# nicolaivicol/otto-recommender

Measured on AMD Instinct MI355X. Metric: co-visit pairs/sec + candidates/sec at 220M events, 1/2/4/8 MI355X, higher is better.
Workload: dtype int32; 1 GPU; configs[1]: all 5 co-visitation rules, 220M events, 100k-session files; events=220000079, sessions=13435907, parallelism=files dealt over 1 GPU(s)

## Files before the change

otto-recommender_amd/csrc/abi.hip:

```cpp
#include <cstdarg>
#include <cstdlib>
#include <ctime>
#include <algorithm>
#include <mutex>
#include "prims.h"
#include "covis_kernels.h"
#include "table.h"

using namespace ottohip;

namespace ottohip {
static thread_local char g_err[1024] = "";
void set_error(const char* fmt, ...) {
  va_list ap;
  va_start(ap, fmt);
  vsnprintf(g_err, sizeof g_err, fmt, ap);
  va_end(ap);
}
}

namespace ottohip {
Ctx* ctx_base(ottohip_ctx* c) { return c; }

int ensure_part_stats(const ottohip_table* tc) {
// ... 743 lines not shown
    s2 = ctx->aux;
  }
  const char* pipe_env = getenv("OTTOHIP_SPLIT_PIPE");
  const bool pipe_on = pipe_env && atoi(pipe_env) == 1;
  const char* sched_env = getenv("OTTOHIP_REDUCE_SCHED");
  const bool sched = s2 != nullptr && sched_env && atoi(sched_env) == 1 && !pipe_on && !lds_leaf &&
                     getenv("OTTOHIP_HASH_PROF") == nullptr;
  auto level_err = [&](int set) { return sched ? reinterpret_cast<int*>(lcount + set * LC_WORDS + LC_ERR) : err; };
  hipMemsetAsync(lcount, 0, 2 * LC_WORDS * 8, s);
  k_classify_rows<<<grid_for(Rn), 256, 0, s>>>(row_begin, Rn, P, Lt.WB, TL, level_err(0), row_base);
  const char* hgrid_env = getenv("OTTOHIP_HASH_GRID");
  const int hgrid = hgrid_env ? std::max(0, atoi(hgrid_env)) : -1;
  const int fom = FOhist ? 2 : (FOmir ? 3 : (FOon ? 1 : 0));
  unsigned int* hnext = nullptr;
  if (hgrid != 0) OH_TRY(ws.get("hash_next", 2, &hnext));
  if (hgrid < 0 && !ctx->hash_resident[fom]) {
    int nb = 0;
    hipError_t e = fom == 2   ? hipOccupancyMaxActiveBlocksPerMultiprocessor(&nb, k_agg_hash<2>, AGG_T, 0)
                   : fom == 3 ? hipOccupancyMaxActiveBlocksPerMultiprocessor(&nb, k_agg_hash<3>, AGG_T, 0)
                   : fom == 1 ? hipOccupancyMaxActiveBlocksPerMultiprocessor(&nb, k_agg_hash<1>, AGG_T, 0)
                              : hipOccupancyMaxActiveBlocksPerMultiprocessor(&nb, k_agg_hash<0>, AGG_T, 0);
    if (e != hipSuccess || nb < 1) { set_error("k_agg_hash<%d>: occupancy query failed", fom); return OTTOHIP_EHIP; }
    ctx->hash_resident[fom] = nb * ctx->n_cu;
  }
  bool srcA = true;
  bool drained = false;
  const bool dbg = getenv("OTTOHIP_DEBUG") != nullptr;
  if (dbg) fprintf(stderr, "[ottohip] P=%llu rows=%lld\n", (unsigned long long)P, (long long)Rn);
  uint32_t* wcur0 = w0;
  const bool pipe = s2 != nullptr && !lds_leaf && !dbg && getenv("OTTOHIP_HASH_PROF") == nullptr && pipe_on;
  const uint64_t PIPE_MIN_CHUNKS = getenv("OTTOHIP_SPLIT_PIPE_MIN") ? (uint64_t)atoll(getenv("OTTOHIP_SPLIT_PIPE_MIN")) : 2048;
  unsigned long long done[N_LISTS] = {};
  bool hash_early = false;
  auto launch_hash_range = [&](uint64_t lo, uint64_t hi, uint32_t* wb0, hipStream_t st, Task* ov,
                               unsigned long long* n_ov, unsigned long long* ov_work, int slot) {
    if (hi <= lo) return;
    const int64_t nh = (int64_t)(hi - lo);
    const Task* th = TL.hash + lo;
    const int64_t blocks = hgrid == 0 ? (int64_t)agg_grid : (hgrid > 0 ? (int64_t)hgrid : (int64_t)ctx->hash_resident[fom]);
    const unsigned hg = (unsigned)std::min<int64_t>(nh, blocks);
    unsigned int* nt = hgrid == 0 ? nullptr : hnext + slot;
    if (nt) hipMemsetAsync(nt, 0, sizeof(unsigned int), st);
    if (FOhist)
      k_agg_hash<2><<<hg, AGG_T, 0, st>>>(th, nh, wb0, w1, row_key, R, Lt, n_rules, O, ov, n_ov, fo, nt, ov_work);
    else if (FOmir)
      k_agg_hash<3><<<hg, AGG_T, 0, st>>>(th, nh, wb0, w1, row_key, R, Lt, n_rules, O, ov, n_ov, fo, nt, ov_work);
    else if (FOon)
      k_agg_hash<1><<<hg, AGG_T, 0, st>>>(th, nh, wb0, w1, row_key, R, Lt, n_rules, O, ov, n_ov, fo, nt, ov_work);
    else
      k_agg_hash<<<hg, AGG_T, 0, st>>>(th, nh, wb0, w1, row_key, R, Lt, n_rules, O, ov, n_ov, fo, nt, ov_work);
  };
  auto launch_sorts = [&](const unsigned long long* lo, const unsigned long long* hi, uint32_t* wb0, hipStream_t st) {
    const unsigned sgrid = (unsigned)ctx->n_cu * 32;
#define OH_SORT(c, M)                                                                                          \
    if (hi[c] > lo[c]) {                                                                                       \
      const int64_t n_ = (int64_t)(hi[c] - lo[c]);                                                             \
      const Task* t_ = TL.sort[c] + lo[c];                                                                     \
      const unsigned g_ = (unsigned)std::min<uint64_t>(ceil_div(n_, 4), sgrid);                                \
      if (FOhist)                                                                                              \
        k_agg_sort<M, 2><<<g_, 256, (size_t)fo.nf * 8, st>>>(t_, n_, wb0, w1, row_key, R, Lt, n_rules, Osort, fo); \
      else if (FOmir)                                                                                          \
        k_agg_sort<M, 3><<<g_, 256, 0, st>>>(t_, n_, wb0, w1, row_key, R, Lt, n_rules, Osort, fo);             \
      else if (FOon)                                                                                           \
        k_agg_sort<M, 1><<<g_, 256, 0, st>>>(t_, n_, wb0, w1, row_key, R, Lt, n_rules, Osort, fo);             \
      else                                                                                                     \
        k_agg_sort<M><<<g_, 256, 0, st>>>(t_, n_, wb0, w1, row_key, R, Lt, n_rules, Osort, fo);                \
    }
    OH_SORT(0, 1) OH_SORT(1, 2) OH_SORT(2, 4) OH_SORT(3, 8) OH_SORT(4, 16)
#undef OH_SORT
  };
  static const int sub = getenv("OTTOHIP_SPLIT_SUB") ? atoi(getenv("OTTOHIP_SPLIT_SUB")) : 4096;
  const char* lds_env = getenv("OTTOHIP_SPLIT_LDS");
  const bool split_lds = lds_env ? atoi(lds_env) != 0 : SPLIT_LDS_DEFAULT;
  const char* ldsmin_env = getenv("OTTOHIP_SPLIT_LDS_MIN");
  const uint32_t lds_min = (uint32_t)std::min(SPLIT_CH + 1, std::max(0, ldsmin_env ? atoi(ldsmin_env) : SPLIT_LDS_MIN));
  const int lds_t = getenv("OTTOHIP_SPLIT_LDS_T") ? atoi(getenv("OTTOHIP_SPLIT_LDS_T")) : SPLIT_LT;
  auto scatter_chunks = [&](const Task* cur_split, int64_t ns, const uint64_t* chb, const uint32_t* ctask, const uint64_t* mtb,
                            const uint64_t* hoff, uint32_t* hmat, uint32_t c0, uint32_t c1) {
    if (c1 <= c0) return;
    uint32_t max_len = SPLIT_CH;
    if (split_lds) {
      if (lds_t == 512)
        k_split_scatter_lds<512><<<c1 - c0, 512, 0, s>>>(cur_split, ns, chb, ctask, mtb, hoff, wcur0, w1, Lt.F, hmat, c0, lds_min);
// ... 12 lines not shown
    hipStream_t s3 = ctx->aux2;
    const unsigned long long* hv = ctx->level_host;
    Task* ovl[2] = {nullptr, nullptr};
    bool hash_pending = false;
    for (int level = 0; level < 40; ++level) {
      const int p = level & 1;
      unsigned long long* C = lcount + p * LC_WORDS;
      unsigned long long* Cn = lcount + (p ^ 1) * LC_WORDS;
      wcur0 = (level == 0 || !w2) ? w0 : w2;
      if (hash_pending) OH_HIP(hipStreamWaitEvent(s, ctx->ev_hash, 0));
      hash_pending = false;
      OH_HIP(hipMemcpyAsync(ctx->level_host, C, LC_WORDS * 8, hipMemcpyDeviceToHost, s));
      OH_HIP(hipMemsetAsync(Cn, 0, LC_WORDS * 8, s));
      OH_HIP(hipEventRecord(ctx->ev_fork, s));
      OH_HIP(hipStreamSynchronize(s));
      if (hv[LC_ERR]) {
        set_error("task list overflow / row too large (err=%d)", (int)hv[LC_ERR]);
        return OTTOHIP_ELIMIT;
      }
      unsigned long long nlist[N_LISTS];
      for (int c = 0; c < N_LISTS; ++c) nlist[c] = hv[c];
      const uint64_t nh = nlist[N_SORT], nov = hv[LC_OVERFLOW];
      const int64_t nsl = (int64_t)nlist[N_SORT + 1], ns = nsl + (int64_t)nov;
      const int64_t nchunks = (int64_t)hv[LC_CHUNKS], ndig = (int64_t)hv[LC_DIGITS], nent = (int64_t)hv[LC_ENTRIES];
      if (dbg)
        fprintf(stderr, "[ottohip] level %d: sort %llu/%llu/%llu/%llu/%llu hash %llu split %llu lds %llu overflow %llu "
                "(chunks %lld digits %lld entries %lld)\n", level, nlist[0], nlist[1], nlist[2], nlist[3], nlist[4],
                (unsigned long long)nh, nlist[N_SORT + 1], nlist[N_SORT + 2], (unsigned long long)nov, (long long)nchunks,
                (long long)ndig, (long long)nent);
      if ((uint64_t)nsl > TL.cap) { set_error("split list overflow"); return OTTOHIP_ELIMIT; }
      if (nh) {
        if ((rc = ws.get(p ? "t_overB" : "t_overA", (size_t)nh, &ovl[p]))) return rc;
        OH_HIP(hipStreamWaitEvent(s3, ctx->ev_fork, 0));
        launch_hash_range(0, nh, wcur0, s3, ovl[p], Cn + LC_OVERFLOW, Cn + LC_CHUNKS, 0);
        OH_HIP(hipEventRecord(ctx->ev_hash, s3));
        hash_pending = true;
      }
      OH_HIP(hipStreamWaitEvent(s2, ctx->ev_fork, 0));
      const unsigned long long zero[N_LISTS] = {};
      launch_sorts(zero, nlist, wcur0, s2);
      OH_HIP(hipEventRecord(ctx->ev_join[p], s2));
      if (ns == 0 && !hash_pending) {
        OH_HIP(hipStreamWaitEvent(s, ctx->ev_join[p], 0));
        drained = true;
        return 0;
      }
      Task* cur_split = TL.split;
      uint32_t *nch, *ndg, *nen, *hmat = nullptr;
      uint64_t *chb, *dgb = nullptr, *mtb = nullptr, *tot2, *hoff = nullptr;
      if (ns) {
        if (nov)
          OH_HIP(hipMemcpyAsync(cur_split + nsl, ovl[p ^ 1], (size_t)nov * sizeof(Task), hipMemcpyDeviceToDevice, s));
        uint32_t* ctask;
        if ((rc = ws.get("sp_nch", (size_t)ns, &nch)) || (rc = ws.get("sp_ndg", (size_t)ns, &ndg)) ||
            (rc = ws.get("sp_nen", (size_t)ns, &nen)) || (rc = ws.get("sp_chb", (size_t)ns + 1, &chb)) ||
            (rc = ws.get("sp_dgb", (size_t)ns + 1, &dgb)) || (rc = ws.get("sp_mtb", (size_t)ns + 1, &mtb)) ||
            (rc = ws.get("sp_tot", 6, &tot2)) || (rc = ws.get("sp_hmat", (size_t)nent, &hmat)) ||
            (rc = ws.get("sp_hoff", (size_t)nent + 1, &hoff)) || (rc = ws.get("sp_ctask", (size_t)nchunks, &ctask)))
          return rc;
        k_split_prepare<<<grid_for(ns), 256, 0, s>>>(cur_split, ns, nch, ndg, nen);
        if ((rc = exclusive_scan_u32(ctx, nch, chb, ns, tot2, s)) || (rc = exclusive_scan_u32(ctx, ndg, dgb, ns, tot2 + 1, s)) ||
            (rc = exclusive_scan_u32(ctx, nen, mtb, ns, tot2 + 2, s)))
          return rc;
        k_split_chunk_task<<<grid_for(ns), 256, 0, s>>>(chb, nch, ns, ctask);
        k_split_hist<<<(unsigned)nchunks, SPLIT_T, 0, s>>>(cur_split, ns, chb, ctask, mtb, wcur0, w1, Lt.F, hmat);
        if ((rc = exclusive_scan_u32(ctx, hmat, hoff, nent, hoff + nent, s))) return rc;
        scatter_chunks(cur_split, ns, chb, ctask, mtb, hoff, hmat, 0, (uint32_t)nchunks);
      }
      if (level >= 1) OH_HIP(hipStreamWaitEvent(s, ctx->ev_join[p ^ 1], 0));
      if ((rc = get_lists(std::max(cap0, (uint64_t)ndig), p ? "t_splitA" : "t_splitB", p ^ 1, nh))) return rc;
      TL.n = Cn;
      if (ns) k_split_classify<<<grid_for(ndig), 256, 0, s>>>(cur_split, ns, dgb, mtb, hoff, ndig, TL, level_err(p ^ 1), hmat, 0);
      if (hipGetLastError() != hipSuccess) { set_error("split launch failed"); return OTTOHIP_EHIP; }
    }
    return 0;
  };
  if (sched) OH_TRY(sched_levels());
  for (int level = 0; !sched && level < 40; ++level) {
    wcur0 = (level == 0 || !w2) ? w0 : w2;
    unsigned long long nlist[N_LISTS];
    if ((rc = d2h(nlist, lcount, N_LISTS, s))) return rc;
    if ((rc = d2h(&herr, err, 1, s))) return rc;
    if (herr) { set_error("task list overflow / row too large (err=%d)", herr); return OTTOHIP_ELIMIT; }
    if (dbg) {
      fprintf(stderr, "[ottohip] level %d: sort %llu/%llu/%llu/%llu/%llu hash %llu split %llu lds %llu\n", level, nlist[0],
              nlist[1], nlist[2], nlist[3], nlist[4], nlist[N_SORT], nlist[N_SORT + 1], nlist[N_SORT + 2]);
      Task* lists[N_LISTS] = {TL.sort[0], TL.sort[1], TL.sort[2], TL.sort[3], TL.sort[4], TL.hash, TL.split, TL.lds};
      fprintf(stderr, "[ottohip] level %d words:", level);
      for (int c = 0; c < N_LISTS; ++c) {
        std::vector<Task> tv(nlist[c]);
        if (nlist[c]) (void)d2h(tv.data(), lists[c], nlist[c], s);
        unsigned long long sw = 0, mx = 0;
        for (auto& t : tv) { sw += t.len; mx = std::max<unsigned long long>(mx, t.len); }
        fprintf(stderr, " %llu(max %llu)", sw, mx);
        if (c == N_SORT + 1 && !tv.empty()) {
          unsigned long long hw[40] = {}, hn[40] = {};
          for (auto& t : tv) { const int b = 63 - __builtin_clzll((unsigned long long)t.len | 1ull); hw[b] += t.len; ++hn[b]; }
          fprintf(stderr, " [split by log2 len:");
          for (int b = 0; b < 40; ++b)
            if (hn[b]) fprintf(stderr, " 2^%d:%llu tasks/%llu words", b, hn[b], hw[b]);
          fprintf(stderr, "]");
        }
      }
      fprintf(stderr, "\n");
    }
    hipStream_t ss = s2 ? s2 : s;
    if (s2) { OH_HIP(hipEventRecord(ctx->ev_fork, s)); OH_HIP(hipStreamWaitEvent(s2, ctx->ev_fork, 0)); }
    static const bool hash_first = !(getenv("OTTOHIP_HASH_FIRST") && !strcmp(getenv("OTTOHIP_HASH_FIRST"), "0"));
    const bool hf = hash_first && nlist[N_SORT] > done[N_SORT];
    auto launch_hash = [&]() {
      launch_hash_range(done[N_SORT], nlist[N_SORT], wcur0, s, TL.split, lcount + N_SORT + 1, nullptr, 0);
    };
    if (hf) launch_hash();
    launch_sorts(done, nlist, wcur0, ss);
    if (s2) OH_HIP(hipEventRecord(ctx->ev_join[level & 1], s2));
    if (nlist[N_SORT + 2]) {
      const unsigned lg = (unsigned)std::min<uint64_t>(nlist[N_SORT + 2], (uint64_t)ctx->n_cu * 4);
      if (FOon)
        k_agg_lds<true><<<lg, LDS_T, 0, s>>>(TL.lds, (int64_t)nlist[N_SORT + 2], wcur0, w1, row_key, R, Lt, O, TL.split,
                                             lcount + N_SORT + 1, TL.cap + split_extra, err, fo);
      else
        k_agg_lds<<<lg, LDS_T, 0, s>>>(TL.lds, (int64_t)nlist[N_SORT + 2], wcur0, w1, row_key, R, Lt, O, TL.split,
                                       lcount + N_SORT + 1, TL.cap + split_extra, err, fo);
    }
    if (nlist[N_SORT] > done[N_SORT]) {
      static const bool hprof = getenv("OTTOHIP_HASH_PROF") != nullptr && !hash_first;
      if (hprof) {
        if ((rc = ws.get("hash_prof", (size_t)(2 * nlist[N_SORT]), &fo.prof))) return rc;
        OH_HIP(hipMemsetAsync(fo.prof, 0, 16 * nlist[N_SORT], s));
      }
      if (!hf) launch_hash();
      if (hprof) {
        std::vector<unsigned long long> pv(2 * nlist[N_SORT]);
        if ((rc = d2h(pv.data(), fo.prof, pv.size(), s))) return rc;
        std::vector<size_t> ord(nlist[N_SORT]);
        for (size_t i = 0; i < ord.size(); ++i) ord[i] = i;
        auto tk = [&](size_t i) { return pv[2 * i + 1] & ~(1ull << 63); };
        std::sort(ord.begin(), ord.end(), [&](size_t a, size_t b) { return tk(a) > tk(b); });
        unsigned long long tsum = 0, wsum = 0;
        for (size_t i = 0; i < ord.size(); ++i) { tsum += tk(i); wsum += (uint32_t)pv[2 * i]; }
        fprintf(stderr, "[ottohip] hash level %d: %zu tasks, %llu words, %.3f ms summed task time; slowest:", level,
                ord.size(), wsum, tsum / 1e5);
        for (size_t i = 0; i < ord.size() && i < 10; ++i)
          fprintf(stderr, " [len %u rows %u %.3f ms%s]", (uint32_t)pv[2 * ord[i]], (uint32_t)(pv[2 * ord[i]] >> 32),
                  tk(ord[i]) / 1e5, (pv[2 * ord[i] + 1] >> 63) ? " full" : "");
        fprintf(stderr, "\n");
        fo.prof = nullptr;
      }
    }
    if (hash_early) OH_HIP(hipStreamWaitEvent(s, ctx->ev_hash, 0));
    if (nlist[N_SORT] || nlist[N_SORT + 2])
      if ((rc = d2h(nlist, lcount, N_LISTS, s))) return rc;
    hash_early = false;
    for (int c = 0; c < N_LISTS; ++c) done[c] = 0;
    const int64_t ns = (int64_t)nlist[N_SORT + 1];
    if (dbg) fprintf(stderr, "[ottohip] level %d: split after hash overflow %lld\n", level, (long long)ns);
    if (ns == 0) {
      if (s2) OH_HIP(hipStreamWaitEvent(s, ctx->ev_join[level & 1], 0));
      drained = true;
      break;
    }
    if ((uint64_t)ns > TL.cap) { set_error("split list overflow"); return OTTOHIP_ELIMIT; }
    Task* cur_split = TL.split;
    uint32_t *nch, *ndg, *nen;
    uint64_t *chb, *dgb, *mtb, *tot2;
    if ((rc = ws.get("sp_nch", (size_t)ns, &nch)) || (rc = ws.get("sp_ndg", (size_t)ns, &ndg)) ||
        (rc = ws.get("sp_nen", (size_t)ns, &nen)) || (rc = ws.get("sp_chb", (size_t)ns + 1, &chb)) ||
        (rc = ws.get("sp_dgb", (size_t)ns + 1, &dgb)) || (rc = ws.get("sp_mtb", (size_t)ns + 1, &mtb)) ||
        (rc = ws.get("sp_tot", 6, &tot2)))
      return rc;
    k_split_prepare<<<grid_for(ns), 256, 0, s>>>(cur_split, ns, nch, ndg, nen);
    if ((rc = exclusive_scan_u32(ctx, nch, chb, ns, tot2, s)) || (rc = exclusive_scan_u32(ctx, ndg, dgb, ns, tot2 + 1, s)) ||
        (rc = exclusive_scan_u32(ctx, nen, mtb, ns, tot2 + 2, s)))
      return rc;
    if (pipe) k_split_half<<<1, 64, 0, s>>>(chb, dgb, ns, tot2, tot2 + 3);
    uint64_t tt[6] = {0, 0, 0, 0, 0, 0};
    if ((rc = d2h(tt, tot2, pipe ? 6 : 3, s))) return rc;
    const int64_t nchunks = (int64_t)tt[0], ndig = (int64_t)tt[1], nent = (int64_t)tt[2];
    const bool piped = pipe && (uint64_t)nchunks >= PIPE_MIN_CHUNKS && tt[3] > 0 && (int64_t)tt[3] < ns &&
                       tt[4] > 0 && (int64_t)tt[4] < nchunks && tt[5] > 0 && (int64_t)tt[5] < ndig;
    const uint32_t cA = piped ? (uint32_t)tt[4] : (uint32_t)nchunks;
    const int64_t dA = piped ? (int64_t)tt[5] : ndig;
    uint32_t *hmat, *ctask;
    uint64_t* hoff;
    if ((rc = ws.get("sp_hmat", (size_t)nent, &hmat)) || (rc = ws.get("sp_hoff", (size_t)nent + 1, &hoff)) ||
        (rc = ws.get("sp_ctask", (size_t)nchunks, &ctask)))
      return rc;
    k_split_chunk_task<<<grid_for(ns), 256, 0, s>>>(chb, nch, ns, ctask);
    k_split_hist<<<(unsigned)nchunks, SPLIT_T, 0, s>>>(cur_split, ns, chb, ctask, mtb, wcur0, w1, Lt.F, hmat);
    if ((rc = exclusive_scan_u32(ctx, hmat, hoff, nent, hoff + nent, s))) return rc;
    auto scatter = [&](uint32_t c0, uint32_t c1) { scatter_chunks(cur_split, ns, chb, ctask, mtb, hoff, hmat, c0, c1); };
    scatter(0, cA);
    if (s2 && level >= 1) OH_HIP(hipStreamWaitEvent(s, ctx->ev_join[(level + 1) & 1], 0));
    const uint64_t capn = (uint64_t)ndig;
    if ((rc = get_lists(std::max(cap0, capn), srcA ? "t_splitB" : "t_splitA", (level + 1) & 1))) return rc;
    hipMemsetAsync(lcount, 0, LC_WORDS * 8, s);
    k_split_classify<<<grid_for(dA), 256, 0, s>>>(cur_split, ns, dgb, mtb, hoff, dA, TL, err, hmat, 0);
    if (piped) {
      if (getenv("OTTOHIP_SPLIT_PIPE_LOG")) fprintf(stderr, "[ottohip] level %d split pipelined at chunk %u of %lld\n", level, cA, (long long)nchunks);
      OH_HIP(hipEventRecord(ctx->ev_half, s));
      scatter(cA, (uint32_t)nchunks);
      if (ndig > dA)
        k_split_classify<<<grid_for(ndig - dA), 256, 0, s>>>(cur_split, ns, dgb, mtb, hoff, ndig, TL, err, hmat, dA);
      OH_HIP(hipStreamWaitEvent(ctx->aux2, ctx->ev_half, 0));
      unsigned long long nA[N_LISTS];
      if ((rc = d2h(nA, lcount, N_LISTS, ctx->aux2))) return rc;
      OH_HIP(hipStreamWaitEvent(s2, ctx->ev_half, 0));
      uint32_t* wb0 = w2 ? w2 : w0;
      if (nA[N_SORT]) {
        launch_hash_range(0, nA[N_SORT], wb0, s2, TL.split, lcount + N_SORT + 1, nullptr, 1);
        OH_HIP(hipEventRecord(ctx->ev_hash, s2));
        hash_early = true;
      }
      const unsigned long long zero[N_LISTS] = {};
      launch_sorts(zero, nA, wb0, s2);
      for (int c = 0; c <= N_SORT; ++c) done[c] = nA[c];
    }
    srcA = !srcA;
    if (hipGetLastError() != hipSuccess) { set_error("split launch failed"); return OTTOHIP_EHIP; }
  }
  ctx->end(ph, s);
  if (!drained) { set_error("reduce: split levels did not converge"); return OTTOHIP_ELIMIT; }
  std::vector<unsigned long long> stv((size_t)STAT_STRIPES * STAT_STRIDE);
  if ((rc = d2h(stv.data(), stats, stv.size(), s))) return rc;
  unsigned long long st[STAT_STRIDE] = {};
  for (int k = 0; k < STAT_STRIPES; ++k)
    for (int j = 0; j < STAT_STRIDE; ++j) st[j] += stv[(size_t)k * STAT_STRIDE + j];
  if (hipGetLastError() != hipSuccess) { set_error("reduce failed"); return OTTOHIP_EHIP; }
  unsigned long long U = 0, dropped = 0;
  for (int r = 0; r < n_rules; ++r) U += st[r * 4 + 0];
  const unsigned long long sum_pairs = st[STAT_RAW + 1], raw_rows = st[STAT_RAW];
  if (FOon) {
    if ((rc = d2h(&dropped, fo.dropped, 1, s))) return rc;
    if (fo.dbg) {
      unsigned long long dv[8];
      if ((rc = d2h(dv, fo.dbg, 8, s))) return rc;
      fprintf(stderr, "[ottohip] file opts: hash dropped %llu kept %llu (loaded %llu inserted %llu), sort dropped %llu kept %llu\n",
              dv[0], dv[1], dv[4], dv[5], dv[2], dv[3]);
    }
    if ((rc = file_opts_finish(fopts, fo, s))) return rc;
  }
  T->n_rows = (int64_t)U;
  T->n_slots = (int64_t)n_slots;
// ... 1096 lines not shown
```

otto-recommender_amd/csrc/covis_kernels.h:

```cpp
#pragma once
#include "prims.h"

namespace ottohip {

constexpr int EV_BLOCK = 256;
constexpr int LCAP = 512;
constexpr int SPLIT_MEAN = 420;
constexpr int LDS_SPLIT_MEAN = 2560;
__constant__ uint32_t c_split_mean = SPLIT_MEAN;
__constant__ uint32_t c_split_runs = 0;
__constant__ uint32_t c_split_fuse = 1;
__constant__ uint32_t c_hash_prio = 0;
__constant__ uint32_t c_lds_leaf = 0;
constexpr uint32_t W_EMPTY = 0xFFFFFFFFu;
constexpr int STAT_STRIPES = 256;
constexpr int STAT_RAW = MAX_RULES * 4;
constexpr int STAT_STRIDE = STAT_RAW + 8;

struct RulesDev {
  int32_t lo[MAX_RULES], hi[MAX_RULES];
  uint32_t mask[MAX_RULES];
  int32_t n_of_type[4];
  int32_t rule_of_type[4][MAX_RULES];
  uint32_t sym_mask;
// ... 2196 lines not shown
    }
  }
  return created;
}

constexpr int N_SORT = 5;
constexpr int SORT_MAX = 64 << (N_SORT - 1);
constexpr int LDS_CAP = 4096;
struct TaskLists {
  Task* sort[N_SORT];
  Task* hash;
  Task* split;
  Task* lds;
  unsigned long long* n;
  uint64_t cap;
};
constexpr int N_LISTS = N_SORT + 3;
constexpr int LC_CHUNKS = N_LISTS, LC_DIGITS = N_LISTS + 1, LC_ENTRIES = N_LISTS + 2, LC_OVERFLOW = N_LISTS + 3,
              LC_ERR = N_LISTS + 4, LC_WORDS = 16;
static_assert(LC_ERR < LC_WORDS, "counter set");
__device__ __forceinline__ uint32_t split_ndig_len(uint64_t len);
__device__ __forceinline__ void split_work(uint64_t len, uint32_t& nch, uint32_t& nd) {
  nch = (uint32_t)((len + 16383ull) / 16384ull);
  nd = split_ndig_len(len);
}

template <int FOM = 0>
__global__ __launch_bounds__(AGG_T, 2) void k_agg_hash(const Task* __restrict__ tasks, int64_t n_tasks,
                                                    const uint32_t* __restrict__ w0, const uint32_t* __restrict__ w1,
                                                    const uint32_t* __restrict__ row_key, RulesDev R, Layout L,
                                                    int n_rules, OutRows O, Task* __restrict__ overflow,
                                                    unsigned long long* __restrict__ n_overflow, FileOpts fo,
                                                    unsigned int* __restrict__ next_task = nullptr,
                                                    unsigned long long* __restrict__ ov_work = nullptr) {
  __shared__ unsigned long long lds[2 * HCAP];
  __shared__ unsigned int s_next;
  __shared__ uint32_t wtot[AGG_T / 64];
  __shared__ uint32_t nocc;
  constexpr bool FO = FOM != 0, PM = FOM == 1 || FOM == 3;
  __shared__ unsigned long long fh[FO ? FO_MAXF : 1];
  __shared__ std::conditional_t<PM, PartLds, char> sP[1];
  const int tid = threadIdx.x;
  if (c_hash_prio == 1) __builtin_amdgcn_s_setprio(1);
  else if (c_hash_prio >= 2) __builtin_amdgcn_s_setprio(3);
  RuleAcc acc;
  acc.zero();
  if constexpr (FO) {
    for (uint32_t i = tid; i < fo.nf; i += AGG_T) fh[i] = 0;
    if constexpr (PM) part_lds_load(fo, sP[0]);
    __syncthreads();
  }
  const bool pmode = PM && fo.parts;
  auto take_task = [&](int64_t prev) -> int64_t {
    if (!next_task) return prev < 0 ? (int64_t)blockIdx.x : prev + (int64_t)gridDim.x;
    __syncthreads();
    if (tid == 0) s_next = atomicAdd(next_task, 1u);
    __syncthreads();
    return (int64_t)s_next;
  };
  for (int64_t ti = take_task(-1); ti < n_tasks; ti = take_task(ti)) {
    const Task T = tasks[ti];
    const uint64_t t_start = fo.prof ? wall_clock64() : 0;
    const uint32_t* W = (T.buf ? w1 : w0) + T.begin;
    const RowInfo ri = row_info(row_key, T.row, L.A);
    const bool fo_row = FO && ri.type == fo.type;
    const bool fo_cut = fo_row && (fo.cuts || fo.qonly);
    uint32_t ndrop = 0, dbg_loaded = 0, dbg_ins = 0;
    const uint32_t dbound = T.len;
    const bool optimistic = 2 * dbound > (uint32_t)HCAP;
    uint32_t cap = 64;
    while (cap < 2 * dbound && cap < (uint32_t)HCAP) cap <<= 1;
    const uint32_t cm = cap - 1, limit = (uint32_t)HCAP / 4;
    unsigned long long* A = lds;
    for (uint32_t i = tid; i < cap; i += AGG_T) A[i] = SLOT_EMPTY;
    if (tid == 0) nocc = 0;
    __syncthreads();
    bool full = false;
    constexpr int PF = 8;
    uint32_t wbuf[PF], nbuf[PF];
    const uint32_t l64 = (uint32_t)tid & 63u;
#pragma unroll
    for (int j = 0; j < PF; ++j) {
      const uint32_t i = j * AGG_T + tid;
      nbuf[j] = i < T.len ? W[i] : W_EMPTY;
    }
    for (uint32_t i0 = 0; i0 < T.len && !full; i0 += AGG_T * PF) {
#pragma unroll
      for (int j = 0; j < PF; ++j) {
        wbuf[j] = nbuf[j];
        const uint32_t i = i0 + (uint32_t)(AGG_T * PF) + j * AGG_T + tid;
        nbuf[j] = i < T.len ? W[i] : W_EMPTY;
      }
#pragma unroll
      for (int j = 0; j < PF; ++j) {
        if (FO && fo.dbg && wbuf[j] != W_EMPTY) ++dbg_loaded;
        if constexpr (PM) {
          const bool dr = fo_cut && fo_drop(fo, wbuf[j], ri.aid, L);
          ndrop += dr ? 1u : 0u;
          wbuf[j] = dr ? W_EMPTY : wbuf[j];
        }
      }
      if (optimistic && __hip_atomic_load(&nocc, __ATOMIC_RELAXED, __HIP_MEMORY_SCOPE_WORKGROUP) > limit) {
        full = true;
        break;
      }
      uint32_t inc[PF], slot[PF];
#pragma unroll
      for (int j = 0; j < PF; ++j) {
        const uint32_t w = wbuf[j];
        const bool head = l64 == 0u || lane_prev(w) != w;
        const uint64_t hm = __ballot(head);
        const uint64_t after = l64 == 63u ? 0ull : hm & (~0ull << (l64 + 1u));
        const uint32_t end = after ? (uint32_t)__builtin_ctzll(after) : 64u;
        inc[j] = end - l64;
        wbuf[j] = head ? w : W_EMPTY;
      }
      const uint32_t created = hash_insert_batch<PF>(A, wbuf, inc, cm, slot);
      if (FO && fo.dbg) {
#pragma unroll
        for (int j = 0; j < PF; ++j) dbg_ins += (wbuf[j] != W_EMPTY && slot[j] != HASH_FULL) ? inc[j] : 0u;
      }
#pragma unroll
      for (int j = 0; j < PF; ++j) full |= wbuf[j] != W_EMPTY && slot[j] == HASH_FULL;
      if (optimistic) {
        const uint32_t nc = wave_sum(created);
        if (nc && (tid & 63) == 0) atomicAdd(&nocc, nc);
      }
    }
    full = __syncthreads_or(full);
    if (full) {
      if (tid == 0) {
        const unsigned long long k = atomicAdd(n_overflow, 1ull);
        overflow[k] = T;
        if (ov_work) {
          uint32_t nch, nd;
          split_work(T.len, nch, nd);
          atomicAdd(ov_work + 0, (unsigned long long)nch);
          atomicAdd(ov_work + 1, (unsigned long long)nd);
          atomicAdd(ov_work + 2, (unsigned long long)nch * nd);
        }
        if (fo.prof) {
          fo.prof[2 * ti] = T.len;
          fo.prof[2 * ti + 1] = (wall_clock64() - t_start) | (1ull << 63);
        }
      }
      __syncthreads();
      continue;
    }
    constexpr int SL = HCAP / AGG_T;
    uint32_t kw[SL], kc[SL];
#pragma unroll
    for (int s = 0; s < SL; ++s) {
      const uint32_t slot = tid + s * AGG_T;
      const unsigned long long v = slot < cap ? A[slot] : SLOT_EMPTY;
      kw[s] = (uint32_t)(v >> 32);
      kc[s] = (uint32_t)v;
    }
    if constexpr (FO) {
      const uint32_t nd = wave_sum(ndrop);
      if (nd && (tid & 63) == 0) atomicAdd(fo.dropped, (unsigned long long)nd);
      if (fo.dbg) {
        uint32_t kept = 0;
#pragma unroll
        for (int s = 0; s < SL; ++s) kept += kw[s] != W_EMPTY ? kc[s] : 0u;
        kept = wave_sum(kept);
        const uint32_t ld = wave_sum(dbg_loaded), ins = wave_sum(dbg_ins);
        if ((tid & 63) == 0) {
          atomicAdd(fo.dbg + 0, (unsigned long long)nd); atomicAdd(fo.dbg + 1, (unsigned long long)kept);
          atomicAdd(fo.dbg + 4, (unsigned long long)ld); atomicAdd(fo.dbg + 5, (unsigned long long)ins);
        }
      }
      if (fo.hist && fo_row) {
#pragma unroll
        for (int s = 0; s < SL; ++s)
          if (kw[s] != W_EMPTY && (kw[s] >> (L.A + L.F)) == fo.q) {
            const unsigned long long mult = (fo.sym && ((kw[s] >> L.F) & L.amask) != (uint32_t)ri.aid) ? 2ull : 1ull;
            atomicAdd(&fh[kw[s] & ((1u << L.F) - 1u)], mult * (kc[s] >= 2 ? (1ull | (1ull << 32)) : 1ull));
          }
      }
    }
    __syncthreads();
    const int npass = (FOM == 3 && pmode && fo.mirror_off) ? 2 : 1;
    uint32_t nout = 0;
#pragma unroll 1
    for (int pass = 0; pass < npass; ++pass) {
    unsigned long long* B = lds;
    unsigned long long* B2 = lds + cap;
    for (uint32_t i = tid; i < cap; i += AGG_T) { B[i] = SLOT_EMPTY; B2[i] = 0; }
    __syncthreads();
#pragma unroll
    for (int s0 = 0; s0 < SL; s0 += 8) {
      if ((uint32_t)(s0 * AGG_T) >= cap) break;
      uint32_t k2[8], c8[8], slot[8];
#pragma unroll
      for (int j = 0; j < 8; ++j) {
        k2[j] = kw[s0 + j] == W_EMPTY ? W_EMPTY : kw[s0 + j] >> L.F;
        if constexpr (PM) {
          if (pmode && kw[s0 + j] != W_EMPTY) {
            const uint32_t w = kw[s0 + j], f = w & ((1u << L.F) - 1u), ci = sP[0].cut_of[f];
            const uint64_t ka = (uint64_t)(uint32_t)ri.aid, kb = (uint64_t)((w >> L.F) & L.amask);
            const uint64_t key = pass ? ((kb << 32) | ka) : ((ka << 32) | kb);
            k2[j] |= ((uint32_t)sP[0].part_of[f] +
                      ((ci != FO_NOCUT && key >= sP[0].cut_key[ci & (FO_MAXCUT - 1)]) ? 1u : 0u)) << 24;
          }
        }
        c8[j] = kc[s0 + j];
      }
      hash_insert_batch<8>(B, k2, c8, cm, slot);
#pragma unroll
      for (int j = 0; j < 8; ++j) {
        if (slot[j] == HASH_FULL) continue;
        const uint32_t c = c8[j];
        atomicAdd(&B2[slot[j]], ((unsigned long long)(c >= 2 ? c : 0u) << 32) | 1ull | ((c >= 2 ? 1ull : 0ull) << 16));
      }
    }
    __syncthreads();
    uint32_t mine = 0;
    for (uint32_t i = tid; i < cap; i += AGG_T) {
      const uint32_t k2 = (uint32_t)(B[i] >> 32);
      mine += k2 != W_EMPTY && !(pass && (int32_t)(k2 & L.amask) == ri.aid);
    }
    const uint32_t incl = wave_incl_scan(mine);
    if ((tid & 63) == 63) wtot[tid >> 6] = incl;
    __syncthreads();
    uint32_t pre = 0;
    for (int k = 0; k < (tid >> 6); ++k) pre += wtot[k];
    const uint64_t base = T.begin + (pass ? fo.mirror_off : 0ull);
    uint64_t p = base + pre + incl - mine;
    for (uint32_t i = tid; i < cap; i += AGG_T) {
      const unsigned long long v = B[i];
      const uint32_t k2 = (uint32_t)(v >> 32);
      if (k2 == W_EMPTY) continue;
      const unsigned long long v2 = B2[i];
      const int rule = pmode ? 0 : R.rule_of_type[ri.type][k2 >> L.A];
      const uint32_t c = (uint32_t)v, c2 = (uint32_t)(v2 >> 32), nf = (uint32_t)v2;
      const int32_t next = (int32_t)(k2 & L.amask);
      if (pass) {
        if (next != ri.aid) put_row(O, p++, (int)(k2 >> 24), next, ri.aid, c, c2);
        continue;
      }
      const bool mr = rule_sym(R, rule) && next != ri.aid;
      put_row(O, p++, pmode ? (int)(k2 >> 24) : rule, ri.aid, next, c, c2);
      acc.add(rule, c, nf, mr ? 2u : 1u);
    }
    const uint32_t no = wtot[0] + wtot[1] + wtot[2] + wtot[3];
    for (uint32_t i = no + tid; i < T.len; i += AGG_T) O.rule[base + i] = 0xFF;
    if (pass == 0) nout = no;
    __syncthreads();
    }
    if (fo.prof && tid == 0) {
      fo.prof[2 * ti] = T.len | ((unsigned long long)nout << 32);
      fo.prof[2 * ti + 1] = wall_clock64() - t_start;
    }
  }
  acc.flush(O.stats, n_rules);
  if constexpr (FO) {
    if (fo.hist) {
      __syncthreads();
      for (uint32_t i = tid; i < fo.nf; i += AGG_T)
        if (fh[i]) atomicAdd(&fo.hist[i], fh[i]);
    }
  }
}


constexpr int SPLIT_LEVELS = 4;
__device__ __forceinline__ int task_class(uint64_t len, uint32_t level, bool split) {
  for (int c = 0; c < N_SORT; ++c)
    if (len <= (uint64_t)(64 << c)) return c;
  if (split && c_lds_leaf && len <= (uint64_t)LDS_CAP && level < (uint32_t)SPLIT_LEVELS) return N_SORT + 2;
  return (split && level < (uint32_t)SPLIT_LEVELS) ? N_SORT + 1 : N_SORT;
}
__device__ __forceinline__ void push_task_block(const TaskLists& TL, bool valid, uint64_t begin, uint64_t len,
                                                uint32_t row, uint32_t rem, uint32_t buf, bool split, int* err) {
  __shared__ uint32_t bcnt[N_LISTS];
  __shared__ unsigned long long bbase[N_LISTS];
  __shared__ unsigned long long bwork[3];
  if (valid && len > 0xFFFFFFFFull) { atomicOr(err, 2); valid = false; }
  const int c = valid ? task_class(len, rem, split) : -1;
  if (threadIdx.x < N_LISTS) bcnt[threadIdx.x] = 0;
  if (threadIdx.x < 3) bwork[threadIdx.x] = 0;
  __syncthreads();
  uint32_t my = 0;
#pragma unroll
  for (int q = 0; q < N_LISTS; ++q) {
    const uint64_t m = __ballot(c == q);
    if (!m) continue;
    uint32_t wb = 0;
    if (mbcnt(m) == 0 && c == q) wb = atomicAdd(&bcnt[q], (uint32_t)__popcll(m));
    wb = __shfl(wb, __ffsll((long long)m) - 1);
    if (c == q) my = wb + mbcnt(m);
    if (q == N_SORT + 1) {
      uint32_t nch = 0, nd = 0;
      if (c == q) split_work(len, nch, nd);
// ... 311 lines not shown
    for (uint32_t q = 0; q < (tid >> 6); ++q) pre += wsum[q];
    const uint32_t st = pre + incl - v;
    if (own) g = T.begin + st;
    if (tid < (uint32_t)SPLIT_DMAX) { cur[tid] = st; delta[tid] = g - st; }
  }
  __syncthreads();
  for (uint32_t i0 = 0; i0 < m; i0 += 8 * TB) {
    uint32_t wr[8];
#pragma unroll
    for (int j = 0; j < 8; ++j) {
      const uint32_t i = i0 + tid + j * TB;
      wr[j] = i < m ? Win[i] : 0u;
    }
#pragma unroll
    for (int j = 0; j < 8; ++j) {
      const bool valid = i0 + tid + j * TB < m;
      const uint32_t d = split_digit(wr[j], F, T.rem, nd);
      uint32_t slot;
      if (c_split_runs) slot = lds_add_runs(cur, d, valid);
      else slot = valid ? atomicAdd(&cur[d], 1u) : 0u;
      if (valid && slot < (uint32_t)SPLIT_CH) stage[slot] = wr[j];
    }
  }
  __syncthreads();
  for (uint32_t p = tid; p < m; p += TB) {
    const uint32_t w = stage[p];
    Wout[delta[split_digit(w, F, T.rem, nd)] + p] = w;
  }
}

__global__ void k_split_classify(const Task* __restrict__ tasks, int64_t n, const uint64_t* __restrict__ digit_base,
                                 const uint64_t* __restrict__ mat_base, const uint64_t* __restrict__ hoff,
                                 int64_t n_digits_total, TaskLists TL, int* err, const uint32_t* __restrict__ hmat,
                                 int64_t d0 = 0) {
  const int64_t i = d0 + (int64_t)blockIdx.x * blockDim.x + threadIdx.x;
  Task T;
  T.begin = 0; T.rem = 0; T.row = 0; T.buf = 0; T.len = 0;
  uint64_t b = 0, c = 0;
  if (i < n_digits_total) {
    const int64_t t = find_task(digit_base, n, (uint64_t)i);
    T = tasks[t];
    const uint64_t d = (uint64_t)i - digit_base[t], nch = (uint64_t)ceil_div((int64_t)T.len, SPLIT_CH);
    const uint64_t mb = mat_base[t];
    if (nch == 1 && c_split_fuse) {
      uint64_t lo = 0;
      for (uint64_t e = 0; e < d; ++e) lo += hmat[mb + e];
      c = hmat[mb + d];
      b = T.begin + lo;
    } else {
      const uint64_t lo = hoff[mb + d * nch], hi = hoff[mb + (d + 1) * nch];
      c = hi - lo;
      b = T.begin + (lo - hoff[mb]);
    }
  }
  const bool again = c != 0 && (uint64_t)c <= 4 * ((uint64_t)T.len / split_ndig(T) + 1);
  push_task_block(TL, c != 0, b, c, T.row, T.rem + 1u, T.buf ^ 1u, again, err);
}

constexpr int LDS_T = 256;
constexpr int LDS_WPT = LDS_CAP / LDS_T;
constexpr int LDS_SUBW = 32;
constexpr int LDS_NSUB = LDS_CAP / LDS_SUBW;
constexpr int LDS_SEG = 384;
constexpr int LDS_BIG = 128;
static_assert(LDS_SEG + LDS_BIG <= 512, "a grouped segment fits the 512-word fold");
static_assert(LDS_NSUB <= 128, "sub-bucket scan over waves 0 and 1");
template <bool FO = false>
__global__ __launch_bounds__(LDS_T) void k_agg_lds(const Task* __restrict__ tasks, int64_t n_tasks,
                                                   uint32_t* __restrict__ w0, uint32_t* __restrict__ w1,
                                                   const uint32_t* __restrict__ row_key, RulesDev R, Layout L,
                                                   OutRows O, Task* __restrict__ overflow,
                                                   unsigned long long* __restrict__ n_overflow, uint64_t ov_cap,
                                                   int* __restrict__ err, FileOpts fo) {
  __shared__ uint32_t words[LDS_CAP];
  __shared__ uint32_t sh[LDS_NSUB], ss[LDS_NSUB + 1], seg[LDS_NSUB + 1];
  __shared__ uint32_t wtot[LDS_T / 64], nseg;
  __shared__ unsigned long long sacc[LDS_T / 64][STAT_STRIDE];
  __shared__ RulesDev sR;
  __shared__ uint32_t stg[LDS_T / 64][2][64 * 8 + 64];
  __shared__ unsigned long long fh[FO ? FO_MAXF : 1];
  __shared__ std::conditional_t<FO, PartLds, char> sP[1];
  const int tid = threadIdx.x, wv = tid >> 6;
  const uint32_t l = lane_id();
  if (tid == 0) sR = R;
  for (int i = (int)l; i < STAT_STRIDE; i += 64) sacc[wv][i] = 0;
  if constexpr (FO) {
    for (uint32_t i = tid; i < fo.nf; i += LDS_T) fh[i] = 0;
    part_lds_load(fo, sP[0]);
// ... 803 lines not shown
```

Baseline: 98.09 billion pairs/s.

## Size hash tables to task occupancy, prefetch next hash task, add optional task ordering

```diff
diff --git a/otto-recommender_amd/csrc/abi.hip b/otto-recommender_amd/csrc/abi.hip
--- a/otto-recommender_amd/csrc/abi.hip
+++ b/otto-recommender_amd/csrc/abi.hip
@@ -799,23 +799,40 @@
   const uint64_t PIPE_MIN_CHUNKS = getenv("OTTOHIP_SPLIT_PIPE_MIN") ? (uint64_t)atoll(getenv("OTTOHIP_SPLIT_PIPE_MIN")) : 2048;
   unsigned long long done[N_LISTS] = {};
   bool hash_early = false;
+  const bool hot_hash = getenv("OTTOHIP_HOT_HASH") && !strcmp(getenv("OTTOHIP_HOT_HASH"), "1");
+  const bool hash_order = getenv("OTTOHIP_HASH_ORDER") && !strcmp(getenv("OTTOHIP_HASH_ORDER"), "1");
   auto launch_hash_range = [&](uint64_t lo, uint64_t hi, uint32_t* wb0, hipStream_t st, Task* ov,
-                               unsigned long long* n_ov, unsigned long long* ov_work, int slot) {
-    if (hi <= lo) return;
+                               unsigned long long* n_ov, unsigned long long* ov_work, int slot) -> int {
+    if (hi <= lo) return 0;
     const int64_t nh = (int64_t)(hi - lo);
     const Task* th = TL.hash + lo;
+    const uint32_t* trk = nullptr;
     const int64_t blocks = hgrid == 0 ? (int64_t)agg_grid : (hgrid > 0 ? (int64_t)hgrid : (int64_t)ctx->hash_resident[fom]);
+    if (hash_order && nh > blocks) {
+      Task* sorted;
+      uint32_t* srk;
+      unsigned int* cls;
+      if (int r = ws.get(slot ? "hash_sorted1" : "hash_sorted0", (size_t)nh, &sorted)) return r;
+      if (int r = ws.get(slot ? "hash_rk1" : "hash_rk0", (size_t)nh, &srk)) return r;
+      if (int r = ws.get(slot ? "hash_cls1" : "hash_cls0", 64, &cls)) return r;
+      hipMemsetAsync(cls, 0, 64 * sizeof(unsigned int), st);
+      k_hash_classes<<<grid_for(nh), HORD_T, 0, st>>>(th, nh, cls);
+      k_hash_order<<<grid_for(nh), HORD_T, 0, st>>>(th, nh, row_key, cls, cls + 32, sorted, srk);
+      th = sorted;
+      trk = srk;
+    }
     const unsigned hg = (unsigned)std::min<int64_t>(nh, blocks);
     unsigned int* nt = hgrid == 0 ? nullptr : hnext + slot;
     if (nt) hipMemsetAsync(nt, 0, sizeof(unsigned int), st);
     if (FOhist)
-      k_agg_hash<2><<<hg, AGG_T, 0, st>>>(th, nh, wb0, w1, row_key, R, Lt, n_rules, O, ov, n_ov, fo, nt, ov_work);
+      k_agg_hash<2><<<hg, AGG_T, 0, st>>>(th, nh, wb0, w1, row_key, R, Lt, n_rules, O, ov, n_ov, fo, nt, ov_work, trk);
     else if (FOmir)
-      k_agg_hash<3><<<hg, AGG_T, 0, st>>>(th, nh, wb0, w1, row_key, R, Lt, n_rules, O, ov, n_ov, fo, nt, ov_work);
+      k_agg_hash<3><<<hg, AGG_T, 0, st>>>(th, nh, wb0, w1, row_key, R, Lt, n_rules, O, ov, n_ov, fo, nt, ov_work, trk);
     else if (FOon)
-      k_agg_hash<1><<<hg, AGG_T, 0, st>>>(th, nh, wb0, w1, row_key, R, Lt, n_rules, O, ov, n_ov, fo, nt, ov_work);
+      k_agg_hash<1><<<hg, AGG_T, 0, st>>>(th, nh, wb0, w1, row_key, R, Lt, n_rules, O, ov, n_ov, fo, nt, ov_work, trk);
     else
-      k_agg_hash<<<hg, AGG_T, 0, st>>>(th, nh, wb0, w1, row_key, R, Lt, n_rules, O, ov, n_ov, fo, nt, ov_work);
+      k_agg_hash<<<hg, AGG_T, 0, st>>>(th, nh, wb0, w1, row_key, R, Lt, n_rules, O, ov, n_ov, fo, nt, ov_work, trk);
+    return 0;
   };
   auto launch_sorts = [&](const unsigned long long* lo, const unsigned long long* hi, uint32_t* wb0, hipStream_t st) {
     const unsigned sgrid = (unsigned)ctx->n_cu * 32;
@@ -894,7 +911,7 @@
       if (nh) {
         if ((rc = ws.get(p ? "t_overB" : "t_overA", (size_t)nh, &ovl[p]))) return rc;
         OH_HIP(hipStreamWaitEvent(s3, ctx->ev_fork, 0));
-        launch_hash_range(0, nh, wcur0, s3, ovl[p], Cn + LC_OVERFLOW, Cn + LC_CHUNKS, 0);
+        if ((rc = launch_hash_range(0, nh, wcur0, s3, ovl[p], Cn + LC_OVERFLOW, Cn + LC_CHUNKS, 0))) return rc;
         OH_HIP(hipEventRecord(ctx->ev_hash, s3));
         hash_pending = true;
       }
@@ -932,7 +949,7 @@
       if (level >= 1) OH_HIP(hipStreamWaitEvent(s, ctx->ev_join[p ^ 1], 0));
       if ((rc = get_lists(std::max(cap0, (uint64_t)ndig), p ? "t_splitA" : "t_splitB", p ^ 1, nh))) return rc;
       TL.n = Cn;
-      if (ns) k_split_classify<<<grid_for(ndig), 256, 0, s>>>(cur_split, ns, dgb, mtb, hoff, ndig, TL, level_err(p ^ 1), hmat, 0);
+      if (ns) k_split_classify<<<grid_for(ndig), 256, 0, s>>>(cur_split, ns, dgb, mtb, hoff, ndig, TL, level_err(p ^ 1), hmat, 0, hot_hash);
       if (hipGetLastError() != hipSuccess) { set_error("split launch failed"); return OTTOHIP_EHIP; }
     }
     return 0;
@@ -970,10 +987,10 @@
     if (s2) { OH_HIP(hipEventRecord(ctx->ev_fork, s)); OH_HIP(hipStreamWaitEvent(s2, ctx->ev_fork, 0)); }
     static const bool hash_first = !(getenv("OTTOHIP_HASH_FIRST") && !strcmp(getenv("OTTOHIP_HASH_FIRST"), "0"));
     const bool hf = hash_first && nlist[N_SORT] > done[N_SORT];
-    auto launch_hash = [&]() {
-      launch_hash_range(done[N_SORT], nlist[N_SORT], wcur0, s, TL.split, lcount + N_SORT + 1, nullptr, 0);
+    auto launch_hash = [&]() -> int {
+      return launch_hash_range(done[N_SORT], nlist[N_SORT], wcur0, s, TL.split, lcount + N_SORT + 1, nullptr, 0);
     };
-    if (hf) launch_hash();
+    if (hf && (rc = launch_hash())) return rc;
     launch_sorts(done, nlist, wcur0, ss);
     if (s2) OH_HIP(hipEventRecord(ctx->ev_join[level & 1], s2));
     if (nlist[N_SORT + 2]) {
@@ -991,7 +1008,7 @@
         if ((rc = ws.get("hash_prof", (size_t)(2 * nlist[N_SORT]), &fo.prof))) return rc;
         OH_HIP(hipMemsetAsync(fo.prof, 0, 16 * nlist[N_SORT], s));
       }
-      if (!hf) launch_hash();
+      if (!hf && (rc = launch_hash())) return rc;
       if (hprof) {
         std::vector<unsigned long long> pv(2 * nlist[N_SORT]);
         if ((rc = d2h(pv.data(), fo.prof, pv.size(), s))) return rc;
@@ -1007,6 +1024,12 @@
           fprintf(stderr, " [len %u rows %u %.3f ms%s]", (uint32_t)pv[2 * ord[i]], (uint32_t)(pv[2 * ord[i]] >> 32),
                   tk(ord[i]) / 1e5, (pv[2 * ord[i] + 1] >> 63) ? " full" : "");
         fprintf(stderr, "\n");
+        unsigned long long nsm = 0, tsm = 0;
+        for (size_t i = 0; i < ord.size(); ++i)
+          if ((uint32_t)pv[2 * i] <= 2048u) { ++nsm; tsm += tk(i); }
+        if (nsm)
+          fprintf(stderr, "[ottohip] hash level %d: tasks of <= 2048 words: %llu, %.3f ms summed, %.2f us per task\n", level,
+                  nsm, tsm / 1e5, tsm / 1e2 / (double)nsm);
         fo.prof = nullptr;
       }
     }
@@ -1057,20 +1080,20 @@
     const uint64_t capn = (uint64_t)ndig;
     if ((rc = get_lists(std::max(cap0, capn), srcA ? "t_splitB" : "t_splitA", (level + 1) & 1))) return rc;
     hipMemsetAsync(lcount, 0, LC_WORDS * 8, s);
-    k_split_classify<<<grid_for(dA), 256, 0, s>>>(cur_split, ns, dgb, mtb, hoff, dA, TL, err, hmat, 0);
+    k_split_classify<<<grid_for(dA), 256, 0, s>>>(cur_split, ns, dgb, mtb, hoff, dA, TL, err, hmat, 0, hot_hash);
     if (piped) {
       if (getenv("OTTOHIP_SPLIT_PIPE_LOG")) fprintf(stderr, "[ottohip] level %d split pipelined at chunk %u of %lld\n", level, cA, (long long)nchunks);
       OH_HIP(hipEventRecord(ctx->ev_half, s));
       scatter(cA, (uint32_t)nchunks);
       if (ndig > dA)
-        k_split_classify<<<grid_for(ndig - dA), 256, 0, s>>>(cur_split, ns, dgb, mtb, hoff, ndig, TL, err, hmat, dA);
+        k_split_classify<<<grid_for(ndig - dA), 256, 0, s>>>(cur_split, ns, dgb, mtb, hoff, ndig, TL, err, hmat, dA, hot_hash);
       OH_HIP(hipStreamWaitEvent(ctx->aux2, ctx->ev_half, 0));
       unsigned long long nA[N_LISTS];
       if ((rc = d2h(nA, lcount, N_LISTS, ctx->aux2))) return rc;
       OH_HIP(hipStreamWaitEvent(s2, ctx->ev_half, 0));
       uint32_t* wb0 = w2 ? w2 : w0;
       if (nA[N_SORT]) {
-        launch_hash_range(0, nA[N_SORT], wb0, s2, TL.split, lcount + N_SORT + 1, nullptr, 1);
+        if ((rc = launch_hash_range(0, nA[N_SORT], wb0, s2, TL.split, lcount + N_SORT + 1, nullptr, 1))) return rc;
         OH_HIP(hipEventRecord(ctx->ev_hash, s2));
         hash_early = true;
       }
diff --git a/otto-recommender_amd/csrc/covis_kernels.h b/otto-recommender_amd/csrc/covis_kernels.h
--- a/otto-recommender_amd/csrc/covis_kernels.h
+++ b/otto-recommender_amd/csrc/covis_kernels.h
@@ -2252,7 +2252,8 @@
                                                     int n_rules, OutRows O, Task* __restrict__ overflow,
                                                     unsigned long long* __restrict__ n_overflow, FileOpts fo,
                                                     unsigned int* __restrict__ next_task = nullptr,
-                                                    unsigned long long* __restrict__ ov_work = nullptr) {
+                                                    unsigned long long* __restrict__ ov_work = nullptr,
+                                                    const uint32_t* __restrict__ task_rk = nullptr) {
   __shared__ unsigned long long lds[2 * HCAP];
   __shared__ unsigned int s_next;
   __shared__ uint32_t wtot[AGG_T / 64];
@@ -2271,18 +2272,32 @@
     __syncthreads();
   }
   const bool pmode = PM && fo.parts;
-  auto take_task = [&](int64_t prev) -> int64_t {
-    if (!next_task) return prev < 0 ? (int64_t)blockIdx.x : prev + (int64_t)gridDim.x;
-    __syncthreads();
+  int64_t ti = (int64_t)blockIdx.x, tin = 0;
+  if (next_task) {
     if (tid == 0) s_next = atomicAdd(next_task, 1u);
     __syncthreads();
-    return (int64_t)s_next;
+    ti = (int64_t)s_next;
+    __syncthreads();
+  }
+  Task T, Tn;
+  T.begin = 0; T.len = 0; T.row = 0; T.rem = 0; T.buf = 0;
+  uint32_t rk = 0, rkn = 0;
+  if (ti < n_tasks) {
+    T = tasks[ti];
+    rk = task_rk ? task_rk[ti] : row_key[T.row];
+  }
+  Tn = T;
+  auto advance = [&]() {
+    if (!task_rk && tin < n_tasks) rkn = row_key[Tn.row];
+    ti = tin; T = Tn; rk = rkn;
   };
-  for (int64_t ti = take_task(-1); ti < n_tasks; ti = take_task(ti)) {
-    const Task T = tasks[ti];
+  for (; ti < n_tasks; advance()) {
+    unsigned int nx = 0;
+    if (next_task && tid == 0) nx = atomicAdd(next_task, 1u);
     const uint64_t t_start = fo.prof ? wall_clock64() : 0;
     const uint32_t* W = (T.buf ? w1 : w0) + T.begin;
-    const RowInfo ri = row_info(row_key, T.row, L.A);
+    RowInfo ri;
+    ri.type = (int)(rk >> L.A); ri.aid = (int32_t)(rk & ((1u << L.A) - 1u));
     const bool fo_row = FO && ri.type == fo.type;
     const bool fo_cut = fo_row && (fo.cuts || fo.qonly);
     uint32_t ndrop = 0, dbg_loaded = 0, dbg_ins = 0;
@@ -2347,7 +2362,13 @@
         if (nc && (tid & 63) == 0) atomicAdd(&nocc, nc);
       }
     }
+    if (next_task && tid == 0) s_next = nx;
     full = __syncthreads_or(full);
+    tin = next_task ? (int64_t)s_next : ti + (int64_t)gridDim.x;
+    if (tin < n_tasks) {
+      Tn = tasks[tin];
+      if (task_rk) rkn = task_rk[tin];
+    }
     if (full) {
       if (tid == 0) {
         const unsigned long long k = atomicAdd(n_overflow, 1ull);
@@ -2376,6 +2397,13 @@
       kw[s] = (uint32_t)(v >> 32);
       kc[s] = (uint32_t)v;
     }
+    {
+      uint32_t occ = 0;
+#pragma unroll
+      for (int s = 0; s < SL; ++s) occ += kw[s] != W_EMPTY ? 1u : 0u;
+      occ = wave_sum(occ);
+      if ((tid & 63) == 0) wtot[tid >> 6] = occ;
+    }
     if constexpr (FO) {
       const uint32_t nd = wave_sum(ndrop);
       if (nd && (tid & 63) == 0) atomicAdd(fo.dropped, (unsigned long long)nd);
@@ -2402,11 +2430,15 @@
     __syncthreads();
     const int npass = (FOM == 3 && pmode && fo.mirror_off) ? 2 : 1;
     uint32_t nout = 0;
+    const uint32_t ndw = wtot[0] + wtot[1] + wtot[2] + wtot[3];
+    uint32_t capB = 64;
+    while (capB < 2 * ndw && capB < cap) capB <<= 1;
+    const uint32_t cmB = capB - 1;
 #pragma unroll 1
     for (int pass = 0; pass < npass; ++pass) {
     unsigned long long* B = lds;
-    unsigned long long* B2 = lds + cap;
-    for (uint32_t i = tid; i < cap; i += AGG_T) { B[i] = SLOT_EMPTY; B2[i] = 0; }
+    unsigned long long* B2 = lds + capB;
+    for (uint32_t i = tid; i < capB; i += AGG_T) { B[i] = SLOT_EMPTY; B2[i] = 0; }
     __syncthreads();
 #pragma unroll
     for (int s0 = 0; s0 < SL; s0 += 8) {
@@ -2426,7 +2458,7 @@
         }
         c8[j] = kc[s0 + j];
       }
-      hash_insert_batch<8>(B, k2, c8, cm, slot);
+      hash_insert_batch<8>(B, k2, c8, cmB, slot);
 #pragma unroll
       for (int j = 0; j < 8; ++j) {
         if (slot[j] == HASH_FULL) continue;
@@ -2436,7 +2468,7 @@
     }
     __syncthreads();
     uint32_t mine = 0;
-    for (uint32_t i = tid; i < cap; i += AGG_T) {
+    for (uint32_t i = tid; i < capB; i += AGG_T) {
       const uint32_t k2 = (uint32_t)(B[i] >> 32);
       mine += k2 != W_EMPTY && !(pass && (int32_t)(k2 & L.amask) == ri.aid);
     }
@@ -2447,7 +2479,7 @@
     for (int k = 0; k < (tid >> 6); ++k) pre += wtot[k];
     const uint64_t base = T.begin + (pass ? fo.mirror_off : 0ull);
     uint64_t p = base + pre + incl - mine;
-    for (uint32_t i = tid; i < cap; i += AGG_T) {
+    for (uint32_t i = tid; i < capB; i += AGG_T) {
       const unsigned long long v = B[i];
       const uint32_t k2 = (uint32_t)(v >> 32);
       if (k2 == W_EMPTY) continue;
@@ -2480,6 +2512,67 @@
       for (uint32_t i = tid; i < fo.nf; i += AGG_T)
         if (fh[i]) atomicAdd(&fo.hist[i], fh[i]);
     }
+  }
+}
+
+constexpr int HORD_T = 256;
+__device__ __forceinline__ uint32_t hash_class_place(uint32_t* ctr, uint32_t c, bool valid) {
+  const uint32_t l = threadIdx.x & 63u;
+  uint32_t r = 0;
+  uint64_t todo = __ballot(valid);
+  while (todo) {
+    const uint32_t lead = (uint32_t)__builtin_ctzll(todo);
+    const uint32_t cl = (uint32_t)__shfl((int)c, (int)lead);
+    const bool in_cl = valid && c == cl;
+    const uint64_t m = __ballot(in_cl);
+    uint32_t base = 0;
+    if (l == lead) base = atomicAdd(&ctr[cl], (uint32_t)__builtin_popcountll(m));
+    base = (uint32_t)__shfl((int)base, (int)lead);
+    if (in_cl) r = base + (uint32_t)__builtin_popcountll(m & ((1ull << l) - 1ull));
+    todo &= ~m;
+  }
+  return r;
+}
+__global__ __launch_bounds__(HORD_T) void k_hash_classes(const Task* __restrict__ in, int64_t n,
+                                                         unsigned int* __restrict__ cnt) {
+  __shared__ uint32_t bc[32];
+  const uint32_t tid = threadIdx.x;
+  if (tid < 32) bc[tid] = 0;
+  __syncthreads();
+  const int64_t i = (int64_t)blockIdx.x * HORD_T + tid;
+  const bool valid = i < n;
+  (void)hash_class_place(bc, valid ? 31u - (uint32_t)__builtin_clz(in[i].len | 1u) : 0u, valid);
+  __syncthreads();
+  if (tid < 32 && bc[tid]) atomicAdd(&cnt[tid], bc[tid]);
+}
+__global__ __launch_bounds__(HORD_T) void k_hash_order(const Task* __restrict__ in, int64_t n,
+                                                       const uint32_t* __restrict__ row_key,
+                                                       const unsigned int* __restrict__ cnt,
+                                                       unsigned int* __restrict__ cur, Task* __restrict__ out,
+                                                       uint32_t* __restrict__ out_rk) {
+  __shared__ uint32_t bc[32], bbase[32];
+  const uint32_t tid = threadIdx.x;
+  if (tid < 32) bc[tid] = 0;
+  __syncthreads();
+  const int64_t i = (int64_t)blockIdx.x * HORD_T + tid;
+  const bool valid = i < n;
+  Task T;
+  T.begin = 0; T.len = 0; T.row = 0; T.rem = 0; T.buf = 0;
+  if (valid) T = in[i];
+  const uint32_t rk = valid ? row_key[T.row] : 0u;
+  const uint32_t c = 31u - (uint32_t)__builtin_clz(T.len | 1u);
+  const uint32_t r = hash_class_place(bc, c, valid);
+  __syncthreads();
+  if (tid < 32 && bc[tid]) {
+    uint32_t before = 0;
+    for (uint32_t k = tid + 1; k < 32; ++k) before += cnt[k];
+    bbase[tid] = before + atomicAdd(&cur[tid], bc[tid]);
+  }
+  __syncthreads();
+  if (valid) {
+    const uint32_t p = bbase[c] + r;
+    out[p] = T;
+    out_rk[p] = rk;
   }
 }
 
@@ -2857,7 +2950,7 @@
 __global__ void k_split_classify(const Task* __restrict__ tasks, int64_t n, const uint64_t* __restrict__ digit_base,
                                  const uint64_t* __restrict__ mat_base, const uint64_t* __restrict__ hoff,
                                  int64_t n_digits_total, TaskLists TL, int* err, const uint32_t* __restrict__ hmat,
-                                 int64_t d0 = 0) {
+                                 int64_t d0 = 0, bool hot_hash = false) {
   const int64_t i = d0 + (int64_t)blockIdx.x * blockDim.x + threadIdx.x;
   Task T;
   T.begin = 0; T.rem = 0; T.row = 0; T.buf = 0; T.len = 0;
@@ -2878,7 +2971,9 @@
       b = T.begin + (lo - hoff[mb]);
     }
   }
-  const bool again = c != 0 && (uint64_t)c <= 4 * ((uint64_t)T.len / split_ndig(T) + 1);
+  const bool capped = ((uint64_t)T.len + c_split_mean - 1) / c_split_mean > (uint64_t)SPLIT_DMAX;
+  const bool again = c != 0 && (capped || !hot_hash || c_lds_leaf) &&
+                     (uint64_t)c <= 4 * ((uint64_t)T.len / split_ndig(T) + 1);
   push_task_block(TL, c != 0, b, c, T.row, T.rem + 1u, T.buf ^ 1u, again, err);
 }
 
```

Result: no change. 98.66 billion pairs/s (median of 6 runs) (+0.6%).
